# HKUST-Aerial-Robotics/ESVO

Measured on AMD Instinct MI355X. Metric: mapped events/sec (stereo TS raster + block matching + LM depth refinement + fusion), events resident in HBM before the timed region; exactly K ticks between two synchronisations, i.e. including the fill and the drain of the two-deep tick pipeline (`sustained`: the same workload over 1600 ticks), higher is better.
Workload: dtype f64

## Files before the change

esvo_amd/csrc/api_core.hip:

```cpp
#include "context.hpp"

namespace esvo_host {
thread_local std::string g_create_error;
}

namespace {

void invert3x3(const double* P, double* Kinv, double* Kinv_t) {
  const double a = P[0], b = P[1], cc = P[2], d = P[4], e = P[5], f = P[6], g = P[8], hh = P[9], i = P[10];
  const double det = a * (e * i - f * hh) - b * (d * i - f * g) + cc * (d * hh - e * g);
  const double id = 1.0 / det;
  Kinv[0] = (e * i - f * hh) * id; Kinv[1] = (cc * hh - b * i) * id; Kinv[2] = (b * f - cc * e) * id;
  Kinv[3] = (f * g - d * i) * id;  Kinv[4] = (a * i - cc * g) * id;  Kinv[5] = (cc * d - a * f) * id;
  Kinv[6] = (d * hh - e * g) * id; Kinv[7] = (b * g - a * hh) * id;  Kinv[8] = (a * e - b * d) * id;
  for (int r = 0; r < 3; ++r) Kinv_t[r] = (Kinv[r * 3 + 0] * P[3] + Kinv[r * 3 + 1] * P[7]) + Kinv[r * 3 + 2] * P[11];
}

int validate_params(const esvo_params_t* p, std::string& why) {
  if (p->ls_norm != ESVO_LSNORM_TDIST && p->ls_norm != ESVO_LSNORM_L2) { why = "LSnorm must be Tdist or l2 (DepthProblemSolver.cpp:121-131 exits on anything else)"; return ESVO_ERR_UNSUPPORTED; }
  if (p->bm_step < 1) { why = "BM_step must be >= 1"; return ESVO_ERR_INVALID_ARG; }
  if (p->patch_size_x < 1 || p->patch_size_x > 64 || p->patch_size_y < 1 || p->patch_size_y > 40) { why = "patch size must be within 1..64 x 1..40"; return ESVO_ERR_UNSUPPORTED; }
  if (p->median_blur_kernel_size < 0 || p->median_blur_kernel_size > 3) { why = "median_blur_kernel_size must be 0..3 (kernel 2k + 1)"; return ESVO_ERR_UNSUPPORTED; }
  if (p->max_event_queue_len < 0 || p->max_event_queue_len > TSQ_LMAX) { why = "max_event_queue_len must be 0 (one stamp per pixel) or 1..32"; return ESVO_ERR_UNSUPPORTED; }
  if (p->bm_max_disparity < p->bm_min_disparity || p->bm_min_disparity < 0) { why = "bad disparity range"; return ESVO_ERR_INVALID_ARG; }
// ... 26 lines not shown
  HIPCHK(hipMemsetAsync(h->d_map, 0, map_buffer_bytes(npx), st));
  HIPCHK(hipMemsetAsync(h->d_map2, 0, map_buffer_bytes(npx), st));
  HIPCHK(hipMemsetAsync(h->d_tile_count, 0, sizeof(u32) * fuse_front_tiles(h), st));
  HIPCHK(hipMemsetAsync(h->d_fuse_ctr, 0, sizeof(u32) * 2112, st));
  if (h->d_rank_kept) HIPCHK(hipMemsetAsync(h->d_rank_kept, 0, sizeof(u32) * esvo_context::SHARD_MAX_RANKS, st));
  h->d_map_cur = h->d_map;
  return ESVO_OK;
}

void read_dev_switches(esvo_context* h) {
  const char* e;
  if ((e = esvo_dev_switch("ESVO_LM_PAIR"))) h->lm_pair_forced = std::atoi(e) == 1 ? 1 : (std::atoi(e) == 0 ? 0 : -1);
  if ((e = esvo_dev_switch("ESVO_LM_QUEUES"))) h->lm_queues = std::atoi(e) == 1 ? 1 : (std::atoi(e) == 2 ? 2 : 0);
  if ((e = esvo_dev_switch("ESVO_TIMELINE"))) h->tl_on = std::atoi(e) != 0;
  if ((e = esvo_dev_switch("ESVO_LOWLAT"))) h->lat_mode = std::atoi(e) != 0;
  if ((e = esvo_dev_switch("ESVO_LOWLAT_TIMED_EVERY"))) h->lat_timed_every = std::max(1, std::atoi(e));
  if ((e = esvo_dev_switch("ESVO_REG_SPARSE"))) h->reg_sparse_forced = std::atoi(e) != 0 ? 1 : 0;
  if ((e = esvo_dev_switch("ESVO_PIPE_TIMED_EVERY"))) h->pipe_timed_every = std::max(1, std::atoi(e));
  if ((e = esvo_dev_switch("ESVO_LOWLAT_MAX_EVENTS"))) h->lat_max_events = (u32)std::strtoul(e, nullptr, 10);
  if (h->tsq_len > 0) h->tsq_tcap = (e = esvo_dev_switch("ESVO_TSQ_TILE_CAP")) ? (u32)std::max(1, std::atoi(e)) : 1024u;
  if (h->max_ev > LM_TWO_QUEUES_MAX_EVENTS && (e = esvo_dev_switch("ESVO_LM_ORDER"))) h->lm_order_on = std::atoi(e) != 0;
  if ((e = esvo_dev_switch("ESVO_BM_DEDUPE"))) h->bm_dedupe_on = std::atoi(e) != 0;
  if ((e = esvo_dev_switch("ESVO_BM_DEDUPE_MIN"))) h->bm_dedupe_min = (u32)std::max(1L, std::atol(e));
  if ((e = esvo_dev_switch("ESVO_CLK_PROBE"))) h->clk_probe = std::atoi(e) != 0;
  h->n_pose_slots = (e = esvo_dev_switch("ESVO_POSE_SLOTS0")) ? (u32)std::max(1, std::atoi(e)) : 1024u;
  if ((e = esvo_dev_switch("ESVO_FUSE_TILE_CAP"))) h->fuse_tile_cap = (u32)std::max(1L, std::atol(e));
  if ((e = esvo_dev_switch("ESVO_FUSE_PMAX"))) h->fuse_pmax_plus1 = (u32)std::max(0L, std::atol(e)) + 1u;
  if ((e = esvo_dev_switch("ESVO_FUSE_TILE_REC"))) h->fuse_tile_rec = (u32)std::max(1L, std::atol(e));
  if ((e = esvo_dev_switch("ESVO_FUSE_LDS_CAP"))) h->fuse_lds_cap = (u32)std::max(0L, std::atol(e));
}

int create_streams(esvo_context* h) {
  int prio_lo = 0, prio_hi = 0;
  CK(hipDeviceGetStreamPriorityRange(&prio_lo, &prio_hi));
  CK(hipStreamCreateWithPriority(&h->stream, hipStreamNonBlocking, prio_hi));
  CK(hipStreamCreateWithPriority(&h->stream_b, hipStreamNonBlocking, prio_hi));
  h->own_stream = true;
  CK(hipStreamCreateWithPriority(&h->stream_l, hipStreamNonBlocking, prio_lo));
  CK(hipStreamCreateWithPriority(&h->stream_l1, hipStreamNonBlocking, prio_lo));
  CK(hipStreamCreateWithFlags(&h->stream_t, hipStreamNonBlocking));
  CK(hipStreamCreateWithFlags(&h->stream_i, hipStreamNonBlocking));
  return ESVO_OK;
}

int alloc_camera(esvo_context* h, int cam, const esvo_calib_t* c) {
  const size_t npx = (size_t)h->W * h->H;
// ... 52 lines not shown
  h->d_pose_T = h->pose[0].d_T;
  return ESVO_OK;
}

int alloc_tick_scratch(esvo_context* h) {
  const size_t npx = (size_t)h->W * h->H, E = h->max_ev;
  if (h->max_ev > 4000000u) FAIL(ESVO_ERR_CAPACITY, "max_events_per_tick too large (scan limit 4M)");
  if (npx > 4000000u) FAIL(ESVO_ERR_CAPACITY, "image too large (scan limit 4M pixels)");
  CK(h->d_tick_ev.alloc(E));
  CK(h->d_match_slots.alloc(E));
  CK(h->d_match_flags.alloc(E)); CK(h->d_match_prefix.alloc(E));
  for (int k = 0; k < 2; ++k) CK(h->front[k].d_matches.alloc(E));
  if (E >= LM_SPLIT_MIN_EVENTS) {
    CK(h->d_lm_fvec0.alloc(E * 7 * 16)); CK(h->d_lm_fnorm0.alloc(E));
    CK(h->d_lm_meta.alloc(E)); CK(h->d_lm_order.alloc(E));
    CK(h->d_lm_hist.alloc(2 * 32 * 64));
    CK(hipMemset(h->d_lm_hist, 0, sizeof(u32) * 2 * 32 * 64));
  }
  if (E > LM_TWO_QUEUES_MAX_EVENTS) {
    for (int k = 0; k < 2; ++k) { CK(h->front[k].d_lm_pix_order.alloc(E)); CK(h->d_lm_sort_rows[k].alloc(E)); }
    CK(h->d_lm_sort_hist.alloc(voxel_hist_words(E)));
  }
  if (h->bm_dedupe_on && E >= h->bm_dedupe_min) CK(h->d_bm_dedupe.alloc(npx + 4 + 2 * E));
  CK(h->d_clk.alloc(2 * clk_words(h->max_ev)));
  CK(hipMemset(h->d_clk, 0, sizeof(u64) * 2 * clk_words(h->max_ev)));
  int khz = 0;
  if (hipDeviceGetAttribute(&khz, hipDeviceAttributeWallClockRate, h->device) != hipSuccess || khz <= 0) khz = 100000;
  h->stats.clk_ref_khz = (uint32_t)khz;
  for (int k = 0; k < 2; ++k) {
    CK(h->front[k].d_pt_slots.alloc(E));
    CK(h->front[k].d_pt_flags.alloc(E)); CK(h->front[k].d_pt_prefix.alloc(E));
    CK(h->front[k].d_scan_tmp_l.alloc(scan_scratch_elems(std::max(E, npx)) + 8));
  }
  CK(h->d_pts_tmp.alloc(E));
  for (int k = 0; k < 2; ++k) CK(h->front[k].d_stage.alloc(E));
  for (int k = 0; k < 2; ++k) CK(h->front[k].d_counters.alloc(CNT_ROW));
  for (int k = 0; k < 2; ++k) CK(hipMemset(h->front[k].d_counters, 0, sizeof(u32) * CNT_ROW));
  CK(h->h_counters.alloc(CNT_ROW * 2));
  std::memset(h->h_counters, 0, sizeof(u32) * CNT_ROW * 2);
  CK(h->h_pin.alloc(2 * ((size_t)h->max_poses * 17 + 16)));
  CK(h->d_scan_tmp.alloc(scan_scratch_elems(std::max(E, npx)) + 8)); CK(h->d_scan_tmp_b.alloc(scan_scratch_elems(std::max(E, npx)) + 8));
  CK(h->d_cnt_b.alloc(CNTB_ROW)); CK(hipMemset(h->d_cnt_b, 0, sizeof(u32) * CNTB_ROW));
  CK(h->h_cnt_b.alloc(CNTB_ROW * CNTB_ROWS));
  std::memset(h->h_cnt_b, 0, sizeof(u32) * CNTB_ROW * CNTB_ROWS);
  for (int k = 0; k < 2; ++k) { h->front[k].d_clk = h->d_clk + (size_t)k * clk_words(h->max_ev); h->front[k].h_counters = h->h_counters + CNT_ROW * k; h->back[k].h_cnt = h->h_cnt_b + CNTB_ROW * k; }
  CK(h->d_halo_viol.alloc(2));
// ... 367 lines not shown
```

esvo_amd/csrc/api_dev.hip:

```cpp
#include <vector>

#include "context.hpp"
#include "fdiv.hpp"

namespace {
using esvo::u32;

constexpr size_t GUARD_WORDS = 64;
constexpr size_t GUARD_BYTES = GUARD_WORDS * sizeof(u32);
constexpr u32 GUARD_PATTERN = 0xA55AC33Cu;

struct GBuf {
  uint8_t* base = nullptr;
  size_t bytes = 0;
  bool pinned = false;
  GBuf() = default;
  GBuf(const GBuf&) = delete;
  GBuf& operator=(const GBuf&) = delete;
  ~GBuf() {
    if (!base) return;
    if (pinned) hipHostFree(base);
    else hipFree(base);
  }
  hipError_t make(size_t n, const void* init, bool pin = false) {
// ... 237 lines not shown
  HIPCHK(d_r.make(img_bytes, img.data()));
  for (int k = 0; k < 2; ++k) HIPCHK(d_rows[k].make(max_matches * 8, nullptr));
  HIPCHK(d_hist.make(esvo::voxel_hist_words(max_matches) * 4, nullptr));
  HIPCHK(d_tmp.make(esvo::scan_scratch_elems(esvo::voxel_hist_words(max_matches)) * 4, nullptr));
  HIPCHK(d_order.make(max_matches * 4, order));
  esvo::DevParams dp;
  std::memset(&dp, 0, sizeof(dp));
  dp.W = width; dp.H = height; dp.num_threads = num_threads; dp.updown = updown;
  esvo::u64* const rows[2] = {d_rows[0].ptr<esvo::u64>(), d_rows[1].ptr<esvo::u64>()};
  esvo::launch_lm_pixel_order(d_m.ptr<esvo_match_t>(), d_n.ptr<u32>(), cap, 0, d_l.ptr<uint8_t>(), d_r.ptr<uint8_t>(), dp, rows,
                              d_hist.ptr<u32>(), d_tmp.ptr<u32>(), d_order.ptr<u32>(), st.s);
  DEV_RUN_DONE();
  HIPCHK(d_m.finish(nullptr, &bad));
  HIPCHK(d_n.finish(nullptr, &bad));
  HIPCHK(d_l.finish(nullptr, &bad));
  HIPCHK(d_r.finish(nullptr, &bad));
  for (int k = 0; k < 2; ++k) HIPCHK(d_rows[k].finish(nullptr, &bad));
  HIPCHK(d_hist.finish(nullptr, &bad));
  HIPCHK(d_tmp.finish(nullptr, &bad));
  HIPCHK(d_order.finish(order, &bad));
  DEV_RETURN();
}

int esvo_debug_upload_words(const void* src, size_t bytes, void* dst, uint32_t* zero, uint32_t zero_words, uint32_t n_zero) {
  if (bytes % 4 || (bytes && (!src || !dst)) || n_zero > 256u || (zero ? n_zero > zero_words : n_zero != 0)) return ESVO_ERR_INVALID_ARG;
  DEV_BEGIN();
  GBuf h_src, d_dst, d_zero;
  HIPCHK(h_src.make(bytes, src, true));
  HIPCHK(d_dst.make(bytes, dst));
  if (zero) HIPCHK(d_zero.make((size_t)zero_words * 4, zero));
  esvo::launch_upload_words(h_src.ptr<void>(), d_dst.ptr<void>(), bytes, st.s, zero ? d_zero.ptr<u32>() : nullptr, n_zero);
  DEV_RUN_DONE();
  HIPCHK(h_src.finish(nullptr, &bad));
  HIPCHK(d_dst.finish(dst, &bad));
  if (zero) HIPCHK(d_zero.finish(zero, &bad));
  DEV_RETURN();
}

int esvo_debug_back_prologue(const void* src, size_t bytes, void* dst, const void* a_src, size_t a_bytes, void* a_dst, size_t a_dst_bytes,
                             const void* b_src, size_t b_bytes, void* b_dst, const uint32_t* a_flags, const uint32_t* a_prefix,
                             uint32_t a_slots) {
  if (bytes % 4 || a_bytes % 8 || b_bytes % 8 || a_dst_bytes % 8) return ESVO_ERR_INVALID_ARG;
  if ((bytes && (!src || !dst)) || (a_bytes && !a_src) || (a_dst_bytes && !a_dst) || (b_bytes && (!b_src || !b_dst))) return ESVO_ERR_INVALID_ARG;
  if (a_flags ? (!a_prefix || a_bytes != (size_t)a_slots * sizeof(esvo_depth_point_t)) : (a_dst_bytes != a_bytes)) return ESVO_ERR_INVALID_ARG;
  if (a_flags) {
    for (u32 i = 0; i < a_slots; ++i)
// ... 105 lines not shown
  HIPCHK(hipSetDevice(h->device));
  int rc = flush_pending_tick(h);
  if (rc) return rc;
  rc = drain_lm_and_back(h);
  if (rc) return rc;
  HIPCHK(hipMemcpy(out, h->d_cell_count, sizeof(u32) * n, hipMemcpyDeviceToHost));
  return ESVO_OK;
}

int esvo_debug_bm_owner_count(esvo_handle h, uint32_t* n_owners, int* shared) {
  if (!h || !n_owners || !shared) return ESVO_ERR_INVALID_ARG;
  API_LOCK(h);
  HIPCHK(hipSetDevice(h->device));
  int rc = flush_pending_tick(h);
  if (rc) return rc;
  *n_owners = 0;
  *shared = h->d_bm_dedupe ? 1 : 0;
  if (!h->d_bm_dedupe) return ESVO_OK;
  HIPCHK(hipStreamSynchronize(h->stream));
  HIPCHK(hipMemcpy(n_owners, h->d_bm_dedupe + (size_t)h->W * h->H, sizeof(u32), hipMemcpyDeviceToHost));
  return ESVO_OK;
}

void esvo_debug_live_allocations(size_t out[2]) {
  out[0] = esvo::g_live_allocs.load();
  out[1] = esvo::g_live_bytes.load();
}

int esvo_debug_devmem_selftest(int pinned) { return pinned ? devmem_selftest<true>() : devmem_selftest<false>(); }

}
```

esvo_amd/csrc/api_map.hip:

```cpp
#include "context.hpp"

namespace esvo_host {

u64 lower_bound_sec(const esvo_context* h, int cam, double t) {
  const auto& v = h->ts_host[cam];
  size_t lo = 0, hi = v.size();
  while (lo < hi) {
    size_t mid = (lo + hi) / 2;
    if (ns_to_sec(v[mid]) < t) lo = mid + 1; else hi = mid;
  }
  return h->ring_base[cam] + lo;
}
u64 ros_time_from_sec(double t) {
  long long sec64 = (long long)std::floor(t);
  u32 sec = (u32)sec64;
  u32 nsec = (u32)std::round((t - sec) * 1e9);
  sec += (nsec / 1000000000ul);
  nsec %= 1000000000ul;
  return (u64)sec * 1000000000ull + nsec;
}

int upload_poses(esvo_context* h, const uint64_t* pose_t_ns, const double* pose_T, size_t m, u32* d_zero_row) {
  if (m > h->max_poses) FAIL(ESVO_ERR_CAPACITY, "pose table larger than max_poses_per_tick");
  h->pin_slot ^= 1;
// ... 2 lines not shown
  double* sec = pin + 16 * m;
  for (size_t i = 0; i < m; ++i) sec[i] = ns_to_sec(pose_t_ns[i]);
  std::memcpy(T, pose_T, sizeof(double) * 16 * m);
  h->h_pose_T.assign(pose_T, pose_T + 16 * m);
  h->n_pose = (u32)m;
  h->pose_buf ^= 1;
  h->d_pose_T = h->pose[h->pose_buf].d_T;
  HIPCHK(hipStreamWaitEvent(h->stream, h->pose[h->pose_buf].released, 0));
  h->d_pose_sec = h->d_pose_T + 16 * m;
  launch_upload_words(T, h->d_pose_T, sizeof(double) * 17 * m, h->stream, d_zero_row, CNT_ROW);
  return ESVO_OK;
}

int run_bm(esvo_context* h, const esvo_event_t* d_ev, u64 first, u64 cap, int reverse, u32 n, const u32* sel) {
  FrontSlot& F = h->front_cur();
  BmArgs a;
  a.ev = d_ev; a.n = n; a.ev_first = first; a.ev_cap = cap; a.ev_reverse = reverse; a.sel = sel;
  a.tsL = h->d_obs[0]; a.tsR = h->d_obs[1];
  a.lut = h->d_lut; a.mask = h->d_mask;
  a.pose_sec = h->d_pose_sec; a.n_pose = h->n_pose;
  a.out_slots = h->d_match_slots; a.out_flags = h->d_match_flags;
  a.fail_counters = F.d_counters;
  if (h->stage_events_on) hipEventRecord(F.ev->e[FE_BM0], h->stream);
  if (h->d_bm_dedupe && n >= h->bm_dedupe_min && n <= h->max_ev && !h->sharded && bm_dedupe_applies(a, h->dp)) {
    u32* owner = h->d_bm_dedupe;
    u32* n_uniq = owner + (size_t)h->W * h->H;
    u32* uniq_w = n_uniq + 4;
    launch_bm_match_dedupe(a, h->dp, owner, uniq_w, n_uniq, uniq_w + h->max_ev, h->stream);
  } else {
    launch_bm_match(a, h->dp, h->stream);
  }
  if (h->stage_events_on) hipEventRecord(F.ev->e[FE_BM1], h->stream);
  HIPCHK(hipGetLastError());
  return ESVO_OK;
}
int run_order_matches(esvo_context* h, u32 n, bool local, bool by_index) {
  FrontSlot& F = h->front_cur();
  if (scan_compact_is_small(n)) {
    by_index = by_index && !local;
    launch_scan_compact_matches_small(h->d_match_flags, h->d_match_prefix, F.d_counters + (local ? CNT_OWN_MATCHES : CNT_MATCHES), n, h->d_match_slots,
                                      by_index ? nullptr : F.d_matches, (local || by_index) ? h->d_own_w : nullptr, h->stream);
  } else {
    launch_exclusive_scan_u32(h->d_match_flags, h->d_match_prefix, F.d_counters + (local ? CNT_OWN_MATCHES : CNT_MATCHES), h->d_scan_tmp, n, h->stream);
    launch_compact_matches(h->d_match_slots, h->d_match_flags, h->d_match_prefix, n, F.d_matches, local ? h->d_own_w : nullptr,
                           h->stream);
  }
  if (h->stage_events_on) hipEventRecord(F.ev->e[FE_S1], h->stream);
// ... 594 lines not shown
```

esvo_amd/csrc/common.hpp:

```cpp
#pragma once

#include <hip/hip_runtime.h>
#include <stdint.h>

#include "../../include/esvo_hip.h"

#define ESVO_WAVE 64

#include <cstdlib>
#include <cstring>
inline const char* esvo_dev_switch(const char* name) {
  const char* on = std::getenv("ESVO_DEV_SWITCHES");
  return (on && std::strcmp(on, "1") == 0) ? std::getenv(name) : nullptr;
}

namespace esvo {

typedef unsigned long long u64;
typedef unsigned int u32;

struct CamConst {
  double P[12];
  double Kinv[9];
  double Kinv_t[3];
// ... 154 lines not shown
  u64* q;
  int L;
  u32* tcount; uint4* tlist; u32 tcap;
  uint4* over; u32* over_count; u32 over_cap;
};
void launch_tsq_insert(const TsQueueArgs& a, int W, int H, hipStream_t s);
void launch_tsq_view(const u64* q, int L, int W, int H, u64 t_ns, u64* sae, hipStream_t s);
struct TsPair { const u64* sae[2]; uint8_t* raw[2]; const int2* fixmap[2]; uint8_t* out[2]; uint8_t* out2[2]; };
void launch_ts_scatter_segs(const TsScatterSegs& g, int n_seg, int W, int H, hipStream_t s);
void launch_ts_render_pair(const TsPair& c, int W, int H, u64 t_ns, double decay_sec, int ignore_polarity, int median_k,
                           hipStream_t s, int row0 = 0, int row1 = -1);
void launch_ts_render_forward(const u64* d_sae, const u32* d_off, const u32* d_src, const float2* d_lut, double* d_val,
                              uint8_t* d_raw, uint8_t* d_out, int W, int H, u64 t_ns, double decay_sec, int ignore_polarity,
                              int median_k, hipStream_t s);
void launch_gaussian5_pair(const uint8_t* in0, const uint8_t* in1, uint8_t* out0, uint8_t* out1, int W, int H, hipStream_t s,
                           int row0 = 0, int row1 = -1);
void launch_denoise_flags(const esvo_event_t* ring, u64 first, u64 cap, u32 n, uint8_t* evmap, u32* flags, int W, int H,
                          hipStream_t s);
void launch_denoise_select(const u32* flags, const u32* prefix, u32 n, u32* sel, hipStream_t s);
void launch_denoise_bits_routed(const esvo_event_t* ring, u64 first, u64 cap, u32 n_loc, const u32* gidx, u32 g_first, u32 n, uint8_t* evmap,
                                int W, int H, int band_y0, int band_y1, u32* bits, hipStream_t s);
void launch_denoise_bits_unpack(const u32* blocks, u32 block_words, u32 N, u32 n, u32* flags, hipStream_t s);

struct BmArgs {
  const esvo_event_t* ev;
  u32 n;
  u64 ev_first;
  u64 ev_cap;
  int ev_reverse;
  const u32* sel;
  const uint8_t* tsL;
  const uint8_t* tsR;
  const float2* lut;
  const uint8_t* mask;
  const double* pose_sec;
  u32 n_pose;
  esvo_match_t* out_slots;
  u32* out_flags;
  u32* fail_counters;
  const u32* gidx = nullptr;
  u32 g_first = 0;
  u32 n_loc = 0;
  const u32* keep_flags = nullptr;
  const u32* keep_prefix = nullptr;
  u32 n_raw = 0;
  const u32* uniq_w = nullptr;
  const u32* n_uniq = nullptr;
  u32* search_rec = nullptr;
};
void launch_bm_match(const BmArgs& a, const DevParams& p, hipStream_t s);
constexpr unsigned long long BM_LDS_MAX_BYTES = 160ull * 1024ull;
unsigned long long bm_match_lds_bytes(int wx, int wy, int dmin, int dmax, int step, int updown);
constexpr u32 BM_DEDUPE_MIN_EVENTS = 40001u;
bool bm_dedupe_applies(const BmArgs& a, const DevParams& p);
void launch_bm_match_dedupe(BmArgs a, const DevParams& p, u32* owner, u32* uniq_w, u32* n_uniq, u32* search_rec, hipStream_t s);
void launch_compact_matches(const esvo_match_t* slots, const u32* flags, const u32* prefix, u32 n,
                            esvo_match_t* out, u32* slot_of, hipStream_t s);
void launch_matches_to_points(const esvo_match_t* m, const u32* n_ptr, u32 max_n, esvo_depth_point_t* out, const DevParams& p,
                              hipStream_t s);

struct TrackRef { double T[16]; };
struct TrackPose { double T[16]; double Jc[6]; };
#define TRK_NE_MAX_POSES 4
struct TrackPoseSet { TrackPose p[TRK_NE_MAX_POSES]; };
struct TrackArgs {
  const double* pts;
  const uint8_t* neg;
  const int16_t* du;
  const int16_t* dv;
  const uint8_t* mask;
  double P[12];
  int W, H;
};
void launch_track_images(const uint8_t* blurred, uint8_t* neg, int16_t* du, int16_t* dv, int W, int H, hipStream_t s);
void launch_track_reference(const float* xyz, u32 n, const TrackRef& r, double* pts, hipStream_t s);
void launch_track_reference_gather(const float* cloud_xyz, const u32* order, u32 n, const TrackRef& r, double* pts, hipStream_t s);
void launch_track_residuals(const TrackArgs& a, const TrackPose& pose, u32 offset, u32 count, int huber, double thr, double* fvec,
                            hipStream_t s);
// ... 162 lines not shown
```

esvo_amd/csrc/context.hpp:

```cpp
#pragma once
#include <algorithm>
#include <array>
#include <atomic>
#include <chrono>
#include <cmath>
#include <cstdio>
#include <cstdlib>
#include <cstring>
#include <deque>
#include <mutex>
#include <string>
#include <vector>

#include "common.hpp"
#include "devmem.hpp"

using namespace esvo;

struct FrameRec {
  u32 off;
  u32 count;
  u32 slot;
  u32 run;
};
// ... 165 lines not shown
  DevBuf<uint8_t> d_wire[2];
  u64 ring_cap = 0;
  DevEvent evt_ingest[2];

  DevBuf<uint8_t> d_obs_tmp;

  PoseBuf pose[2];
  int pose_buf = 0;
  std::vector<double> h_pose_T;
  PinBuf<double> h_pin;

  u32 max_ev = 0;
  DevBuf<esvo_event_t> d_tick_ev;
  DevBuf<esvo_match_t> d_match_slots;
  DevBuf<u32> d_match_flags, d_match_prefix;
  DevBuf<double> d_lm_fvec0, d_lm_fnorm0;
  DevBuf<u32> d_lm_meta, d_lm_order, d_lm_hist;
  DevBuf<u64> d_lm_sort_rows[2];
  DevBuf<u32> d_lm_sort_hist;
  bool lm_order_on = true;
  DevBuf<u32> d_bm_dedupe;
  bool bm_dedupe_on = true;
  u32 bm_dedupe_min = esvo::BM_DEDUPE_MIN_EVENTS;
  DevBuf<u64> d_clk;
  bool clk_probe = true;
  DevBuf<DevPoint> d_pts_tmp;
  PinBuf<u32> h_counters;
  DevBuf<u32> d_scan_tmp;
  DevBuf<u32> d_cnt_b;
  PinBuf<u32> h_cnt_b;
  DevBuf<u32> d_scan_tmp_b;

  DevBuf<DevPoint> d_win;
  u32 win_cap = 0;
  u32 n_pose_slots = 0;
  std::vector<char> slot_used;
  DevBuf<double> d_frame_pose_T;
  u32 max_poses = 0;
  DevBuf<u32> d_fr_table;
  PinBuf<u32> h_fr_table;
  u32 max_frames = 0;

  DevBuf<DevPoint> d_prop;
  DevBuf<u32> d_tile_count;
  DevBuf<uint2> d_tile_pts, d_over_pts;
  DevBuf<u32> d_cell_count, d_cell_offset, d_cell_list;
// ... 229 lines not shown
```

esvo_amd/csrc/kernels_bm.hip:

```cpp
#include "common.hpp"
#include "fdiv.hpp"

namespace esvo {

__device__ inline int wave_sum_i32(int v) {
#pragma unroll
  for (int d = 32; d >= 1; d >>= 1) v += __shfl_xor(v, d, ESVO_WAVE);
  return v;
}
__device__ inline long long wave_sum_i64(long long v) {
#pragma unroll
  for (int d = 32; d >= 1; d >>= 1) v += __shfl_xor(v, d, ESVO_WAVE);
  return v;
}

typedef u32 u32x4_a4 __attribute__((ext_vector_type(4), aligned(4)));

struct ZnccLeft {
  double sigl;
  int Sl;
};
__device__ inline double sqrt_var(double v) { return v > 0 ? sqrt_moderate(v) : 0.0; }
__device__ inline ZnccLeft zncc_left(int Sl, int Sll, int N, const Recip& rn2) {
  ZnccLeft z;
  z.Sl = Sl;
  z.sigl = sqrt_var(div_fast((double)(N * Sll - Sl * Sl), rn2)) + 1e-6;
  return z;
}
__device__ inline double zncc_from_moments(const ZnccLeft& zl, int Sr, int Srr, int Slr, int N, const Recip& rn,
                                           const Recip& rn2) {
  const double varr = div_fast((double)(N * Srr - Sr * Sr), rn2);
  const double sigr = sqrt_var(varr) + 1e-6;
  const double cov = div_fast((double)(N * Slr - zl.Sl * Sr), rn);
  Recip rs;
  rs.b = zl.sigl * sigr;
  rs.y = recip_refined(rs.b);
  return 0.5 * (1 - div_fast(div_fast(cov, rs), rn));
}

extern __shared__ __attribute__((aligned(16))) unsigned char bm_smem[];

template <int G>
__device__ inline int grp_sum_i32(int v) {
#pragma unroll
  for (int d = G / 2; d >= 1; d >>= 1) v += __shfl_xor(v, d, G);
  return v;
}

#ifndef BM_BLOCK
#define BM_BLOCK 64
#endif

__device__ inline uint4 load_row15(const u32* ts32, int n_dw, int A) {
  const int a0 = A >> 2;
  const u32 sh = (u32)(A & 3);
  u32 d[5];
#pragma unroll
  for (int j = 0; j < 5; ++j) {
    int idx = a0 + j;
    idx = idx < 0 ? 0 : (idx >= n_dw ? n_dw - 1 : idx);
    d[j] = ts32[idx];
// ... 25 lines not shown
  e = reinterpret_cast<const uint4*>(a.ev)[ei];
}

template <int G>
__device__ inline void grp_argmin(double& best, int& bestd) {
#pragma unroll
  for (int s = G / 2; s >= 1; s >>= 1) {
    const double oc = __shfl_xor(best, s, G);
    const int od = __shfl_xor(bestd, s, G);
    if (od >= 0 && (bestd < 0 || oc < best || (oc == best && od > bestd))) { best = oc; bestd = od; }
  }
}

__device__ inline u32 pose_lower_bound(const BmArgs& a, const uint4& e) {
  const double te = time_to_sec(e.y, e.z);
  u32 lo = 0, hi = a.n_pose;
  while (lo < hi) {
    const u32 mid = (lo + hi) >> 1;
    if (a.pose_sec[mid] < te) lo = mid + 1; else hi = mid;
  }
  return lo;
}

template <int G, bool COARSE, bool UPDOWN>
__global__ void __launch_bounds__(BM_BLOCK) bm_match_kernel(BmArgs a, DevParams p, int RD, int lds_per_event) {
  constexpr int EPB = BM_BLOCK / G;
  const int grp = threadIdx.x / G, l = threadIdx.x % G;
  const u32 pos = blockIdx.x * EPB + grp;
  const u32 n_out = a.gidx ? a.n_loc : a.n;
  u32 w = a.gidx ? pos : pos * (u32)p.ev_nshards + (u32)p.ev_shard;
  if (a.uniq_w) {
    const u32 nu = *a.n_uniq;
    if (blockIdx.x * EPB >= nu) return;
    w = pos < nu ? a.uniq_w[pos] : n_out;
  }
  u32* ldsL = reinterpret_cast<u32*>(bm_smem + grp * lds_per_event);
  u32* ldsR = ldsL + 28;
  const int nd = p.dmax - p.dmin + 1;
  double* cost_row = reinterpret_cast<double*>(ldsR + (UPDOWN ? (nd + 6) * 4 : 7 * RD));

  const int W = p.W, H = p.H;
  constexpr int wx = 15, wy = 7, N = wx * wy, hx = 7, hy = 3;

  bool ok = w < n_out;
  u32 k = 0;
  uint4 e = make_uint4(0, 0, 0, 0);
  if (ok) bm_item(a, p, w, k, e, ok);
  const int ex = e.x & 0xffffu, ey = e.x >> 16;
  double xr = 0, yr = 0;
  int x1 = 0, y1 = 0;
  if (ok) ok = ex < W && ey < H;
  if (ok) {
    const float2 q = a.lut[ey * W + ex];
    xr = (double)q.x;
    yr = (double)q.y;
    ok = !(xr < 0 || xr > (double)(W - 1) || yr < 0 || yr > (double)(H - 1));
    if (a.gidx && ok) { const int yb = (int)floor(yr); ok = yb >= p.band_y0 && yb < p.band_y1; }
  }
  if (ok && a.mask) ok = a.mask[(int)yr * W + (int)xr] > 125;
  if (ok) {
    x1 = (int)floor(xr);
    y1 = (int)floor(yr);
  }
  if (ok) ok = !(x1 - hx < 1 || y1 - hy < 1 || x1 + hx >= W - 1 || y1 + hy >= H - 1);
  int reason = 0;

  int Sl = 0, Sll = 0;
  if (ok) {
    int cnt = 0, sl = 0, sll = 0;
    if (l < wy) {
      const u32* ts32 = reinterpret_cast<const u32*>(a.tsL);
      const int n_dw = (W * H + 3) >> 2;
      const uint4 wv = load_row15(ts32, n_dw, (y1 - hy + l) * W + (x1 - hx));
      *reinterpret_cast<uint4*>(ldsL + l * 4) = wv;
      u32 usl = 0, usll = 0;
      usl = __builtin_amdgcn_udot4(wv.x, 0x01010101u, usl, false);
      usl = __builtin_amdgcn_udot4(wv.y, 0x01010101u, usl, false);
      usl = __builtin_amdgcn_udot4(wv.z, 0x01010101u, usl, false);
      usl = __builtin_amdgcn_udot4(wv.w, 0x01010101u, usl, false);
      usll = __builtin_amdgcn_udot4(wv.x, wv.x, usll, false);
      usll = __builtin_amdgcn_udot4(wv.y, wv.y, usll, false);
      usll = __builtin_amdgcn_udot4(wv.z, wv.z, usll, false);
      usll = __builtin_amdgcn_udot4(wv.w, wv.w, usll, false);
      auto zero_bytes = [](u32 x) {
        return __popc(~(((x & 0x7f7f7f7fu) + 0x7f7f7f7fu) | x | 0x7f7f7f7fu));
      };
      cnt = zero_bytes(wv.x) + zero_bytes(wv.y) + zero_bytes(wv.z) + zero_bytes(wv.w | 0xff000000u);
      sl = (int)usl;
// ... 37 lines not shown
          *reinterpret_cast<uint4*>(ldsR + py * RD + 4 * j4) = v;
        }
      }
    }
  }
  __syncthreads();

  auto cand_valid = [&](int d) {
    if constexpr (UPDOWN) { const int y2 = y1 - d; return !(y2 - hy < 1 || y2 + hy >= H - 1); }
    else { const int x2 = x1 - d; return !(x2 - hx < 1 || x2 + hx >= W - 1); }
  };
  double best = 1.0;
  int bestd = -1;
  if (ok) {
    const Recip rn = make_recip((double)N), rn2 = make_recip((double)N * (double)N);
    const ZnccLeft zl = zncc_left(Sl, Sll, N, rn2);
    u32 L[wy][4];
#pragma unroll
    for (int py = 0; py < wy; ++py) {
      const uint4 v = *reinterpret_cast<const uint4*>(ldsL + py * 4);
      L[py][0] = v.x; L[py][1] = v.y; L[py][2] = v.z; L[py][3] = v.w;
    }
    for (int d = p.dmin + l; d <= p.dmax; d += G) {
      if (!cand_valid(d)) {
        if constexpr (COARSE) cost_row[d - p.dmin] = 1.0;
        continue;
      }
      const int col0 = p.dmax - d;
      u32 sr = 0, srr = 0, slr = 0;
#pragma unroll
      for (int py = 0; py < wy; ++py) {
        u32 w0, w1, w2, w3;
        if constexpr (UPDOWN) {
          const uint4 v = *reinterpret_cast<const uint4*>(ldsR + (col0 + py) * 4);
          w0 = v.x; w1 = v.y; w2 = v.z; w3 = v.w;
        } else {
          const int b = o_row[py] + col0;
          const u32* row = ldsR + py * RD + (b >> 2);
          const u32 sh = (u32)(b & 3);
          const u32 d0 = row[0], d1 = row[1], d2 = row[2], d3 = row[3], d4 = row[4];
          w0 = __builtin_amdgcn_alignbyte(d1, d0, sh);
          w1 = __builtin_amdgcn_alignbyte(d2, d1, sh);
          w2 = __builtin_amdgcn_alignbyte(d3, d2, sh);
          w3 = __builtin_amdgcn_alignbyte(d4, d3, sh) & 0x00ffffffu;
        }
        slr = __builtin_amdgcn_udot4(L[py][0], w0, slr, false);
        slr = __builtin_amdgcn_udot4(L[py][1], w1, slr, false);
        slr = __builtin_amdgcn_udot4(L[py][2], w2, slr, false);
        slr = __builtin_amdgcn_udot4(L[py][3], w3, slr, false);
        sr = __builtin_amdgcn_udot4(w0, 0x01010101u, sr, false);
        sr = __builtin_amdgcn_udot4(w1, 0x01010101u, sr, false);
        sr = __builtin_amdgcn_udot4(w2, 0x01010101u, sr, false);
        sr = __builtin_amdgcn_udot4(w3, 0x01010101u, sr, false);
        srr = __builtin_amdgcn_udot4(w0, w0, srr, false);
        srr = __builtin_amdgcn_udot4(w1, w1, srr, false);
        srr = __builtin_amdgcn_udot4(w2, w2, srr, false);
        srr = __builtin_amdgcn_udot4(w3, w3, srr, false);
      }
      const double cost = zncc_from_moments(zl, (int)sr, (int)srr, (int)slr, N, rn, rn2);
      if constexpr (COARSE) cost_row[d - p.dmin] = cost;
      else if (cost <= best) { best = cost; bestd = d; }
    }
  }
  if constexpr (COARSE) {
    __syncthreads();
    if (ok) {
      const int step = p.step;
      const int nc = (p.dmax - p.dmin) / step + 1;
      for (int j = l; j < nc; j += G) {
        const int d = p.dmin + j * step;
        if (!cand_valid(d)) continue;
        const double c = cost_row[d - p.dmin];
        if (c <= best) { best = c; bestd = d; }
      }
      grp_argmin<G>(best, bestd);
      bool found = bestd >= 0 && bestd - step >= p.dmin && bestd + step <= p.dmin + (nc - 1) * step;
      if (found) found = cost_row[bestd - step - p.dmin] < 1.0 && cost_row[bestd + step - p.dmin] < 1.0 && best < p.zncc_thr;
      if (!found) { ok = false; reason = 2; }
      else {
        const int cd = bestd;
        double fb = 2.0;
        int fd = -1;
// ... 243 lines not shown
    return (unsigned long long)(((N + 7) & ~7LL) + bm_any_strip_bytes(wx, wy, nd, updown != 0) + (coarse ? nd * 8 : 0));
  }
  return (unsigned long long)(bm_15x7_event_bytes(nd, coarse, updown != 0) * (BM_BLOCK / bm_group_width(nd)));
}

template <bool COARSE, bool UPDOWN>
static void launch_bm_any(const BmArgs& a, const DevParams& p, hipStream_t s) {
  const int nd = p.dmax - p.dmin + 1;
  const int strip = (int)bm_any_strip_bytes(p.wx, p.wy, nd, UPDOWN);
  const size_t lds = (size_t)bm_match_lds_bytes(p.wx, p.wy, p.dmin, p.dmax, COARSE ? 2 : 1, UPDOWN);
  const u32 own = a.gidx ? a.n_loc : ((a.n > (u32)p.ev_shard) ? (a.n - (u32)p.ev_shard + (u32)p.ev_nshards - 1) / (u32)p.ev_nshards : 0);
  if (own == 0) return;
  hipLaunchKernelGGL((bm_match_any_kernel<COARSE, UPDOWN>), dim3(own), dim3(64), lds, s, a, p, strip);
}

template <int G, bool COARSE, bool UPDOWN>
static void launch_bm_g(const BmArgs& a, const DevParams& p, int RD, hipStream_t s) {
  const int nd = p.dmax - p.dmin + 1;
  const int per_event = (int)bm_15x7_event_bytes(nd, COARSE, UPDOWN);
  const int epb = BM_BLOCK / G;
  const u32 own = a.gidx ? a.n_loc : ((a.n > (u32)p.ev_shard) ? (a.n - (u32)p.ev_shard + (u32)p.ev_nshards - 1) / (u32)p.ev_nshards : 0);
  if (own == 0) return;
  const u32 blocks = (own + epb - 1) / epb;
  hipLaunchKernelGGL((bm_match_kernel<G, COARSE, UPDOWN>), dim3(blocks), dim3(BM_BLOCK), (size_t)per_event * epb, s, a, p, RD, per_event);
}
template <bool COARSE, bool UPDOWN>
static void launch_bm_mode(int G, const BmArgs& a, const DevParams& p, int RD, hipStream_t s) {
  switch (G) {
    case 64: launch_bm_g<64, COARSE, UPDOWN>(a, p, RD, s); break;
    case 32: launch_bm_g<32, COARSE, UPDOWN>(a, p, RD, s); break;
    case 16: launch_bm_g<16, COARSE, UPDOWN>(a, p, RD, s); break;
    default: launch_bm_g<8, COARSE, UPDOWN>(a, p, RD, s); break;
  }
}

void launch_bm_match(const BmArgs& a, const DevParams& p, hipStream_t s) {
  if (a.n == 0) return;
  const int nd = p.dmax - p.dmin + 1;
  const int RD = (int)bm_strip_dwords(nd);
  const int bestG = bm_group_width(nd);
  const bool coarse = p.step > 1;
  if (p.wx != 15 || p.wy != 7) {
    if (p.updown) { if (coarse) launch_bm_any<true, true>(a, p, s); else launch_bm_any<false, true>(a, p, s); }
    else { if (coarse) launch_bm_any<true, false>(a, p, s); else launch_bm_any<false, false>(a, p, s); }
    return;
  }
  if (p.updown) {
    if (coarse) launch_bm_mode<true, true>(bestG, a, p, RD, s);
    else launch_bm_mode<false, true>(bestG, a, p, RD, s);
  } else {
    if (coarse) launch_bm_mode<true, false>(bestG, a, p, RD, s);
    else launch_bm_mode<false, false>(bestG, a, p, RD, s);
  }
}

__global__ void __launch_bounds__(256) bm_claim_kernel(BmArgs a, DevParams p, u32* __restrict__ owner, u32* __restrict__ n_uniq) {
  const u32 w = blockIdx.x * blockDim.x + threadIdx.x;
  if (w == 0) *n_uniq = 0u;
  if (w >= a.n) return;
  u32 k = 0;
  uint4 e;
  bool ok = true;
  bm_item(a, p, w, k, e, ok);
  const int ex = e.x & 0xffffu, ey = e.x >> 16;
  if (ex < p.W && ey < p.H) atomicMin(owner + ey * p.W + ex, w);
}
__global__ void __launch_bounds__(256) bm_owner_list_kernel(BmArgs a, DevParams p, const u32* __restrict__ owner, u32* __restrict__ uniq_w,
                                                            u32* __restrict__ n_uniq) {
  __shared__ u32 wave_cnt[4];
  __shared__ u32 base;
  const u32 w = blockIdx.x * blockDim.x + threadIdx.x;
  bool own = false;
  if (w < a.n) {
    u32 k = 0;
    uint4 e;
    bool ok = true;
// ... 113 lines not shown
```

esvo_amd/lib.py:

```python
import ctypes as C
import os
import subprocess

import numpy as np

from .abi import (DEPTH_POINT_DTYPE, EM_POSE_FN, ERR_CAPACITY, ERR_INVALID_ARG, ERR_STATE, EVENT_DTYPE, MATCH_DTYPE, CalibStruct, EmSelectionStruct,
                  EmStatsStruct, GpcParamsStruct, GpcStatsStruct, ParamsStruct, SgmStatsStruct, StatsStruct, TRACK_ITER_DTYPE, TRACK_SOLVE_MAX_ITERATIONS,
                  TrackSolveInfoStruct, TrackSolveParamsStruct)

_CSRC = os.path.join(os.path.dirname(os.path.abspath(__file__)), "csrc")
_LIB_PATH = os.environ.get("ESVO_HIP_LIB") or os.path.join(_CSRC, "libesvo_hip.so")
_SOURCES = ["api_core.hip", "api_ts.hip", "api_map.hip", "api_window.hip", "api_modes.hip", "api_shard.hip", "api_out.hip", "api_comm.hip", "api_bag.hip", "api_track.hip", "scan.hip", "kernels_ts.hip", "kernels_bm.hip", "kernels_lm.hip", "kernels_lm_any.hip", "kernels_fuse.hip", "kernels_shard.hip", "kernels_track.hip", "kernels_track_viz.hip", "kernels_viz.hip", "kernels_sgm.hip", "api_em.hip", "kernels_em.hip", "kernels_cloud.hip", "api_dev.hip", "api_gpc.hip", "kernels_voxel.hip", "api_history.hip"]
HIPCC_FLAGS = ["--offload-arch=gfx950", "-O3", "-std=c++17", "-ffp-contract=off", "-fPIC", "-shared",
               "-Wno-unused-value", "-Wno-unused-result", "-ldl"]

SYMBOLS = [
    "esvo_default_params", "esvo_create", "esvo_destroy", "esvo_reset", "esvo_set_params", "esvo_last_error",
    "esvo_set_stream", "esvo_synchronize", "esvo_ts_push_events", "esvo_ts_push_events_async", "esvo_ts_push_wait", "esvo_host_alloc", "esvo_host_free", "esvo_ts_push_event_array", "esvo_ts_render", "esvo_ts_render_forward", "esvo_map_set_observation",
    "esvo_map_match", "esvo_map_set_poses", "esvo_map_refine", "esvo_map_push_frame", "esvo_map_fuse",
    "esvo_map_tick", "esvo_map_tick_bm_only", "esvo_map_fuse_matches_naive", "esvo_map_tick_resident", "esvo_map_get_depth_points", "esvo_map_get_committed", "esvo_map_get_pointcloud_xyz", "esvo_map_get_last_frame",
    "esvo_get_stats", "esvo_shard_set_band", "esvo_shard_set_routing", "esvo_shard_get_rows", "esvo_shard_exchange", "esvo_shard_tick_phase", "esvo_abi_sizes",
    "esvo_map_front", "esvo_map_front_frame", "esvo_map_push_frame_device", "esvo_map_fuse_async",
    "esvo_track_set_current", "esvo_track_get_images", "esvo_track_set_reference", "esvo_track_residuals", "esvo_track_jacobian",
    "esvo_track_normal_equations", "esvo_track_normal_equations_batch", "esvo_track_register", "esvo_track_solve", "esvo_track_sizes",
# ... 370 lines not shown
    n = len(flags)
    prefix, total = _prefilled(n, np.uint32), _prefilled(1, np.uint32)
    out = _prefilled(n, MATCH_DTYPE) if want_out else None
    slot_of = _prefilled(n, np.uint32) if want_slot_of else None
    fn = _dbg_fn("esvo_debug_compact_matches", [C.c_void_p, C.c_size_t] + [C.c_void_p] * 5)
    g = _dbg_rc(fn(flags.ctypes.data, n, slots.ctypes.data, prefix.ctypes.data, total.ctypes.data, _p(out), _p(slot_of)),
                "esvo_debug_compact_matches")
    return dict(prefix=prefix, total=int(total[0]), out=out, slot_of=slot_of, guards=g)


def debug_lm_order(matches, max_matches, width, height, left, right, num_threads=1, updown=False):
    matches = _dbg_array(matches, MATCH_DTYPE, "matches")
    left = _dbg_array(np.asarray(left).reshape(-1), np.uint8, "left", width * height)
    right = _dbg_array(np.asarray(right).reshape(-1), np.uint8, "right", width * height)
    order = _prefilled(max_matches, np.uint32)
    variant = C.c_int(-1)
    fn = _dbg_fn("esvo_debug_lm_order", [C.c_void_p, C.c_size_t, C.c_size_t, C.c_int, C.c_int, C.c_int, C.c_int, C.c_void_p, C.c_void_p,
                                         C.c_void_p, C.c_void_p])
    g = _dbg_rc(fn(matches.ctypes.data if len(matches) else None, len(matches), int(max_matches), int(width), int(height), int(num_threads),
                   1 if updown else 0, left.ctypes.data, right.ctypes.data, order.ctypes.data, C.addressof(variant)), "esvo_debug_lm_order")
    return dict(order=order, variant=int(variant.value), guards=g)


def debug_compact_points(flags, slots, want_out=True, row=None, total_index=0, pinned_row=False):
    flags, slots = _check_compact_args(flags, slots, DEPTH_POINT_DTYPE)
    n = len(flags)
    if row is None and pinned_row:
        raise ValueError("pinned_row needs the device row it mirrors")
    if row is not None:
        row = _dbg_array(row, np.uint32, "row").copy()
        if not 0 <= total_index < len(row) <= 1024:
            raise ValueError("total_index must lie inside the row (at most 1024 words)")
    prefix, total = _prefilled(n, np.uint32), _prefilled(1, np.uint32)
    out = _prefilled(n, DEPTH_POINT_DTYPE) if want_out else None
    row_host = _prefilled(len(row), np.uint32) if pinned_row else None
    fn = _dbg_fn("esvo_debug_compact_points", [C.c_void_p, C.c_size_t] + [C.c_void_p] * 5 + [C.c_uint32, C.c_uint32, C.c_void_p])
    g = _dbg_rc(fn(flags.ctypes.data, n, slots.ctypes.data, prefix.ctypes.data, None if row is not None else total.ctypes.data, _p(out),
                   _p(row), 0 if row is None else len(row), int(total_index), _p(row_host)), "esvo_debug_compact_points")
    return dict(prefix=prefix, total=int(total[0]) if row is None else int(row[total_index]), out=out, row=row, row_host=row_host,
                guards=g)


def debug_upload_words(src, zero_words=None, n_zero=0):
    src = _dbg_array(src, np.uint32, "src")
    if not 0 <= n_zero <= 256 or n_zero > (zero_words or 0):
        raise ValueError("n_zero: at most 256 words, inside the zero buffer")
# ... 441 lines not shown
        st = np.ascontiguousarray(stamps, np.uint64)
        T = np.ascontiguousarray(poses, np.float64).reshape(-1, 16)
        Tw = np.ascontiguousarray(T_world_cam, np.float64).reshape(16)
        self._ck(self.lib.esvo_map_tick_resident(self.h, int(t_ns), Tw.ctypes.data, st.ctypes.data, T.ctypes.data, st.shape[0]))

    def get_map(self):
        n = C.c_size_t(0)
        out = np.zeros(self.W * self.H, DEPTH_POINT_DTYPE)
        self._ck(self.lib.esvo_map_get_depth_points(self.h, out.ctypes.data, out.shape[0], C.byref(n)))
        return out[: n.value].copy()

    def debug_fuse_cell_counts(self):
        out = np.zeros((self.H, self.W), np.uint32)
        fn = _dbg_fn("esvo_debug_fuse_cell_counts", [C.c_void_p, C.c_void_p, C.c_size_t])
        self._ck(fn(self.h, out.ctypes.data, out.size))
        return out

    def debug_bm_owner_count(self):
        n, shared = C.c_uint32(0), C.c_int(0)
        fn = _dbg_fn("esvo_debug_bm_owner_count", [C.c_void_p, C.c_void_p, C.c_void_p])
        self._ck(fn(self.h, C.byref(n), C.byref(shared)))
        return int(n.value) if shared.value else None

    def get_committed_map(self):
        out = np.zeros(self.W * self.H, DEPTH_POINT_DTYPE)
        n, t = C.c_size_t(), C.c_uint64()
        self._ck(self.lib.esvo_map_get_committed(self.h, out.ctypes.data, out.shape[0], C.byref(n), C.byref(t)))
        return out[:n.value].copy(), int(t.value)

    def get_pointcloud(self):
        n = C.c_size_t(0)
        out = np.zeros((self.W * self.H, 3), np.float32)
        self._ck(self.lib.esvo_map_get_pointcloud_xyz(self.h, out.ctypes.data, out.shape[0], C.byref(n)))
        return out[: n.value].copy()

    def map_cloud_build(self):
        n = C.c_size_t(0)
        self._ck(self.lib.esvo_map_cloud_build(self.h, C.byref(n)))
        return int(n.value)

    def map_cloud(self):
        n = C.c_size_t(0)
        self._ck(self.lib.esvo_map_cloud_get(self.h, None, 0, C.byref(n)))
        out = np.zeros((int(n.value), 3), np.float32)
        if n.value:
            self._ck(self.lib.esvo_map_cloud_get(self.h, out.ctypes.data, out.shape[0], C.byref(n)))
# ... 287 lines not shown
```

Baseline: 188.1 million.

## Precompute right-image patch moments per pixel for block matching

Adds a per-pixel kernel that computes each right-image patch's sum and standard deviation once per tick using sliding row sums, and stores them in a 16-byte table. The block-matching kernel then reads one record per candidate disparity, prefetching the next one, instead of recomputing the right-patch sum and sum of squares with udot4 for every event and candidate. This removes redundant per-candidate arithmetic, including a sqrt, at the cost of an extra full-image pass and a 16-byte gather per candidate. It is enabled by default above a minimum event count. The moments kernel hardcodes a 15x7 patch.

```diff
diff --git a/esvo_amd/csrc/api_core.hip b/esvo_amd/csrc/api_core.hip
--- a/esvo_amd/csrc/api_core.hip
+++ b/esvo_amd/csrc/api_core.hip
@@ -72,6 +72,8 @@
   if (h->max_ev > LM_TWO_QUEUES_MAX_EVENTS && (e = esvo_dev_switch("ESVO_LM_ORDER"))) h->lm_order_on = std::atoi(e) != 0;
   if ((e = esvo_dev_switch("ESVO_BM_DEDUPE"))) h->bm_dedupe_on = std::atoi(e) != 0;
   if ((e = esvo_dev_switch("ESVO_BM_DEDUPE_MIN"))) h->bm_dedupe_min = (u32)std::max(1L, std::atol(e));
+  if ((e = esvo_dev_switch("ESVO_BM_MOMENTS"))) h->bm_moments_on = std::atoi(e) != 0;
+  if ((e = esvo_dev_switch("ESVO_BM_MOMENTS_MIN"))) h->bm_moments_min = (u32)std::max(1L, std::atol(e));
   if ((e = esvo_dev_switch("ESVO_CLK_PROBE"))) h->clk_probe = std::atoi(e) != 0;
   h->n_pose_slots = (e = esvo_dev_switch("ESVO_POSE_SLOTS0")) ? (u32)std::max(1, std::atoi(e)) : 1024u;
   if ((e = esvo_dev_switch("ESVO_FUSE_TILE_CAP"))) h->fuse_tile_cap = (u32)std::max(1L, std::atol(e));
@@ -170,6 +172,7 @@
     CK(h->d_lm_sort_hist.alloc(voxel_hist_words(E)));
   }
   if (h->bm_dedupe_on && E >= h->bm_dedupe_min) CK(h->d_bm_dedupe.alloc(npx + 4 + 2 * E));
+  if (h->bm_moments_on && E >= h->bm_moments_min) CK(h->d_bm_rmom.alloc(npx));
   CK(h->d_clk.alloc(2 * clk_words(h->max_ev)));
   CK(hipMemset(h->d_clk, 0, sizeof(u64) * 2 * clk_words(h->max_ev)));
   int khz = 0;
diff --git a/esvo_amd/csrc/api_dev.hip b/esvo_amd/csrc/api_dev.hip
--- a/esvo_amd/csrc/api_dev.hip
+++ b/esvo_amd/csrc/api_dev.hip
@@ -283,6 +283,25 @@
   DEV_RETURN();
 }
 
+int esvo_debug_bm_right_moments(const uint8_t* right, int width, int height, double* sig_r, int32_t* Sr) {
+  if (!right || !sig_r || !Sr || width < 1 || height < 1 || (size_t)width * height > 4000000u) return ESVO_ERR_INVALID_ARG;
+  DEV_BEGIN();
+  GBuf d_r, d_out;
+  const size_t npx = (size_t)width * height, img_bytes = (npx + 3) / 4 * 4;
+  std::vector<uint8_t> img(img_bytes, 0);
+  std::memcpy(img.data(), right, npx);
+  HIPCHK(d_r.make(img_bytes, img.data()));
+  std::vector<esvo::BmRight> rec(npx);
+  for (size_t i = 0; i < npx; ++i) { rec[i].sig_r = sig_r[i]; rec[i].Sr = Sr[i]; rec[i].pad = (int)GUARD_PATTERN; }
+  HIPCHK(d_out.make(npx * sizeof(esvo::BmRight), rec.data()));
+  esvo::launch_bm_right_moments(d_r.ptr<uint8_t>(), width, height, d_out.ptr<esvo::BmRight>(), st.s);
+  DEV_RUN_DONE();
+  HIPCHK(d_r.finish(nullptr, &bad));
+  HIPCHK(d_out.finish(rec.data(), &bad));
+  for (size_t i = 0; i < npx; ++i) { sig_r[i] = rec[i].sig_r; Sr[i] = rec[i].Sr; bad += (rec[i].pad != 0); }
+  DEV_RETURN();
+}
+
 int esvo_debug_upload_words(const void* src, size_t bytes, void* dst, uint32_t* zero, uint32_t zero_words, uint32_t n_zero) {
   if (bytes % 4 || (bytes && (!src || !dst)) || n_zero > 256u || (zero ? n_zero > zero_words : n_zero != 0)) return ESVO_ERR_INVALID_ARG;
   DEV_BEGIN();
@@ -434,6 +453,13 @@
   return ESVO_OK;
 }
 
+int esvo_debug_bm_moments_used(esvo_handle h, int* used) {
+  if (!h || !used) return ESVO_ERR_INVALID_ARG;
+  API_LOCK(h);
+  *used = h->bm_moments_used ? 1 : 0;
+  return ESVO_OK;
+}
+
 void esvo_debug_live_allocations(size_t out[2]) {
   out[0] = esvo::g_live_allocs.load();
   out[1] = esvo::g_live_bytes.load();
diff --git a/esvo_amd/csrc/api_map.hip b/esvo_amd/csrc/api_map.hip
--- a/esvo_amd/csrc/api_map.hip
+++ b/esvo_amd/csrc/api_map.hip
@@ -48,7 +48,13 @@
   a.out_slots = h->d_match_slots; a.out_flags = h->d_match_flags;
   a.fail_counters = F.d_counters;
   if (h->stage_events_on) hipEventRecord(F.ev->e[FE_BM0], h->stream);
-  if (h->d_bm_dedupe && n >= h->bm_dedupe_min && n <= h->max_ev && !h->sharded && bm_dedupe_applies(a, h->dp)) {
+  const bool slice = n <= h->max_ev && !h->sharded && bm_dedupe_applies(a, h->dp);
+  h->bm_moments_used = h->d_bm_rmom && n >= h->bm_moments_min && slice;
+  if (h->bm_moments_used) {
+    launch_bm_right_moments(a.tsR, h->dp.W, h->dp.H, h->d_bm_rmom, h->stream);
+    a.rmom = h->d_bm_rmom;
+  }
+  if (h->d_bm_dedupe && n >= h->bm_dedupe_min && slice) {
     u32* owner = h->d_bm_dedupe;
     u32* n_uniq = owner + (size_t)h->W * h->H;
     u32* uniq_w = n_uniq + 4;
diff --git a/esvo_amd/csrc/common.hpp b/esvo_amd/csrc/common.hpp
--- a/esvo_amd/csrc/common.hpp
+++ b/esvo_amd/csrc/common.hpp
@@ -200,6 +200,12 @@
                                 int W, int H, int band_y0, int band_y1, u32* bits, hipStream_t s);
 void launch_denoise_bits_unpack(const u32* blocks, u32 block_words, u32 N, u32 n, u32* flags, hipStream_t s);
 
+struct alignas(16) BmRight {
+  double sig_r;
+  int Sr;
+  int pad;
+};
+static_assert(sizeof(BmRight) == 16, "one 16-byte load per candidate");
 struct BmArgs {
   const esvo_event_t* ev;
   u32 n;
@@ -225,6 +231,7 @@
   const u32* uniq_w = nullptr;
   const u32* n_uniq = nullptr;
   u32* search_rec = nullptr;
+  const BmRight* rmom = nullptr;
 };
 void launch_bm_match(const BmArgs& a, const DevParams& p, hipStream_t s);
 constexpr unsigned long long BM_LDS_MAX_BYTES = 160ull * 1024ull;
@@ -232,6 +239,8 @@
 constexpr u32 BM_DEDUPE_MIN_EVENTS = 40001u;
 bool bm_dedupe_applies(const BmArgs& a, const DevParams& p);
 void launch_bm_match_dedupe(BmArgs a, const DevParams& p, u32* owner, u32* uniq_w, u32* n_uniq, u32* search_rec, hipStream_t s);
+constexpr u32 BM_MOMENTS_MIN_EVENTS = 40001u;
+void launch_bm_right_moments(const uint8_t* tsR, int W, int H, BmRight* out, hipStream_t s);
 void launch_compact_matches(const esvo_match_t* slots, const u32* flags, const u32* prefix, u32 n,
                             esvo_match_t* out, u32* slot_of, hipStream_t s);
 void launch_matches_to_points(const esvo_match_t* m, const u32* n_ptr, u32 max_n, esvo_depth_point_t* out, const DevParams& p,
diff --git a/esvo_amd/csrc/context.hpp b/esvo_amd/csrc/context.hpp
--- a/esvo_amd/csrc/context.hpp
+++ b/esvo_amd/csrc/context.hpp
@@ -211,6 +211,10 @@
   DevBuf<u32> d_bm_dedupe;
   bool bm_dedupe_on = true;
   u32 bm_dedupe_min = esvo::BM_DEDUPE_MIN_EVENTS;
+  DevBuf<esvo::BmRight> d_bm_rmom;
+  bool bm_moments_on = true;
+  u32 bm_moments_min = esvo::BM_MOMENTS_MIN_EVENTS;
+  bool bm_moments_used = false;
   DevBuf<u64> d_clk;
   bool clk_probe = true;
   DevBuf<DevPoint> d_pts_tmp;
diff --git a/esvo_amd/csrc/kernels_bm.hip b/esvo_amd/csrc/kernels_bm.hip
--- a/esvo_amd/csrc/kernels_bm.hip
+++ b/esvo_amd/csrc/kernels_bm.hip
@@ -37,6 +37,13 @@
   rs.y = recip_refined(rs.b);
   return 0.5 * (1 - div_fast(div_fast(cov, rs), rn));
 }
+__device__ inline double zncc_from_table(const ZnccLeft& zl, int Sr, double sigr, int Slr, int N, const Recip& rn) {
+  const double cov = div_fast((double)(N * Slr - zl.Sl * Sr), rn);
+  Recip rs;
+  rs.b = zl.sigl * sigr;
+  rs.y = recip_refined(rs.b);
+  return 0.5 * (1 - div_fast(div_fast(cov, rs), rn));
+}
 
 extern __shared__ __attribute__((aligned(16))) unsigned char bm_smem[];
 
@@ -108,7 +115,7 @@
   return lo;
 }
 
-template <int G, bool COARSE, bool UPDOWN>
+template <int G, bool COARSE, bool UPDOWN, bool RMOM = false>
 __global__ void __launch_bounds__(BM_BLOCK) bm_match_kernel(BmArgs a, DevParams p, int RD, int lds_per_event) {
   constexpr int EPB = BM_BLOCK / G;
   const int grp = threadIdx.x / G, l = threadIdx.x % G;
@@ -150,6 +157,14 @@
   }
   if (ok) ok = !(x1 - hx < 1 || y1 - hy < 1 || x1 + hx >= W - 1 || y1 + hy >= H - 1);
   int reason = 0;
+  auto rm_index = [&](int d) {
+    const int i = UPDOWN ? (y1 - d) * p.W + x1 : y1 * p.W + (x1 - d);
+    return min(max(i, 0), p.W * p.H - 1);
+  };
+  BmRight rm_next;
+  if constexpr (RMOM) {
+    if (ok) rm_next = a.rmom[rm_index(p.dmin + l)];
+  }
 
   int Sl = 0, Sll = 0;
   if (ok) {
@@ -233,6 +248,11 @@
       L[py][0] = v.x; L[py][1] = v.y; L[py][2] = v.z; L[py][3] = v.w;
     }
     for (int d = p.dmin + l; d <= p.dmax; d += G) {
+      BmRight rm;
+      if constexpr (RMOM) {
+        rm = rm_next;
+        rm_next = a.rmom[rm_index(d + G)];
+      }
       if (!cand_valid(d)) {
         if constexpr (COARSE) cost_row[d - p.dmin] = 1.0;
         continue;
@@ -259,16 +279,20 @@
         slr = __builtin_amdgcn_udot4(L[py][1], w1, slr, false);
         slr = __builtin_amdgcn_udot4(L[py][2], w2, slr, false);
         slr = __builtin_amdgcn_udot4(L[py][3], w3, slr, false);
-        sr = __builtin_amdgcn_udot4(w0, 0x01010101u, sr, false);
-        sr = __builtin_amdgcn_udot4(w1, 0x01010101u, sr, false);
-        sr = __builtin_amdgcn_udot4(w2, 0x01010101u, sr, false);
-        sr = __builtin_amdgcn_udot4(w3, 0x01010101u, sr, false);
-        srr = __builtin_amdgcn_udot4(w0, w0, srr, false);
-        srr = __builtin_amdgcn_udot4(w1, w1, srr, false);
-        srr = __builtin_amdgcn_udot4(w2, w2, srr, false);
-        srr = __builtin_amdgcn_udot4(w3, w3, srr, false);
-      }
-      const double cost = zncc_from_moments(zl, (int)sr, (int)srr, (int)slr, N, rn, rn2);
+        if constexpr (!RMOM) {
+          sr = __builtin_amdgcn_udot4(w0, 0x01010101u, sr, false);
+          sr = __builtin_amdgcn_udot4(w1, 0x01010101u, sr, false);
+          sr = __builtin_amdgcn_udot4(w2, 0x01010101u, sr, false);
+          sr = __builtin_amdgcn_udot4(w3, 0x01010101u, sr, false);
+          srr = __builtin_amdgcn_udot4(w0, w0, srr, false);
+          srr = __builtin_amdgcn_udot4(w1, w1, srr, false);
+          srr = __builtin_amdgcn_udot4(w2, w2, srr, false);
+          srr = __builtin_amdgcn_udot4(w3, w3, srr, false);
+        }
+      }
+      double cost;
+      if constexpr (RMOM) cost = zncc_from_table(zl, rm.Sr, rm.sig_r, (int)slr, N, rn);
+      else cost = zncc_from_moments(zl, (int)sr, (int)srr, (int)slr, N, rn, rn2);
       if constexpr (COARSE) cost_row[d - p.dmin] = cost;
       else if (cost <= best) { best = cost; bestd = d; }
     }
@@ -558,7 +582,10 @@
   const u32 own = a.gidx ? a.n_loc : ((a.n > (u32)p.ev_shard) ? (a.n - (u32)p.ev_shard + (u32)p.ev_nshards - 1) / (u32)p.ev_nshards : 0);
   if (own == 0) return;
   const u32 blocks = (own + epb - 1) / epb;
-  hipLaunchKernelGGL((bm_match_kernel<G, COARSE, UPDOWN>), dim3(blocks), dim3(BM_BLOCK), (size_t)per_event * epb, s, a, p, RD, per_event);
+  if (a.rmom)
+    hipLaunchKernelGGL((bm_match_kernel<G, COARSE, UPDOWN, true>), dim3(blocks), dim3(BM_BLOCK), (size_t)per_event * epb, s, a, p, RD, per_event);
+  else
+    hipLaunchKernelGGL((bm_match_kernel<G, COARSE, UPDOWN>), dim3(blocks), dim3(BM_BLOCK), (size_t)per_event * epb, s, a, p, RD, per_event);
 }
 template <bool COARSE, bool UPDOWN>
 static void launch_bm_mode(int G, const BmArgs& a, const DevParams& p, int RD, hipStream_t s) {
@@ -588,6 +615,52 @@
     if (coarse) launch_bm_mode<true, false>(bestG, a, p, RD, s);
     else launch_bm_mode<false, false>(bestG, a, p, RD, s);
   }
+}
+
+constexpr int BM_RM_ROWS = 8;
+__global__ void __launch_bounds__(64) bm_right_moments_kernel(const uint8_t* __restrict__ tsR, int W, int H, BmRight* __restrict__ out) {
+  constexpr int N = 15 * 7, hx = 7, hy = 3, K = BM_RM_ROWS;
+  const int x = blockIdx.x * 64 + threadIdx.x, y0 = blockIdx.y * K;
+  if (x >= W) return;
+  const u32* ts32 = reinterpret_cast<const u32*>(tsR);
+  const int n_dw = (W * H + 3) >> 2;
+  int hs[K + 6], hq[K + 6];
+#pragma unroll
+  for (int r = 0; r < K + 6; ++r) {
+    const uint4 wv = load_row15(ts32, n_dw, (y0 - hy + r) * W + (x - hx));
+    u32 s = 0, q = 0;
+    s = __builtin_amdgcn_udot4(wv.x, 0x01010101u, s, false);
+    s = __builtin_amdgcn_udot4(wv.y, 0x01010101u, s, false);
+    s = __builtin_amdgcn_udot4(wv.z, 0x01010101u, s, false);
+    s = __builtin_amdgcn_udot4(wv.w, 0x01010101u, s, false);
+    q = __builtin_amdgcn_udot4(wv.x, wv.x, q, false);
+    q = __builtin_amdgcn_udot4(wv.y, wv.y, q, false);
+    q = __builtin_amdgcn_udot4(wv.z, wv.z, q, false);
+    q = __builtin_amdgcn_udot4(wv.w, wv.w, q, false);
+    hs[r] = (int)s;
+    hq[r] = (int)q;
+  }
+  const Recip rn2 = make_recip((double)N * (double)N);
+  const bool x_ok = !(x - hx < 1 || x + hx >= W - 1);
+#pragma unroll
+  for (int i = 0; i < K; ++i) {
+    const int y = y0 + i;
+    if (y >= H) break;
+    int Sr = 0, Srr = 0;
+#pragma unroll
+    for (int k = 0; k < 7; ++k) { Sr += hs[i + k]; Srr += hq[i + k]; }
+    const double sig = sqrt_var(div_fast((double)(N * Srr - Sr * Sr), rn2)) + 1e-6;
+    const bool valid = x_ok && !(y - hy < 1 || y + hy >= H - 1);
+    BmRight r;
+    r.sig_r = valid ? sig : 0.0;
+    r.Sr = valid ? Sr : 0;
+    r.pad = 0;
+    out[(size_t)y * W + x] = r;
+  }
+}
+void launch_bm_right_moments(const uint8_t* tsR, int W, int H, BmRight* out, hipStream_t s) {
+  if (W < 1 || H < 1) return;
+  hipLaunchKernelGGL(bm_right_moments_kernel, dim3((W + 63) / 64, (H + BM_RM_ROWS - 1) / BM_RM_ROWS), dim3(64), 0, s, tsR, W, H, out);
 }
 
 __global__ void __launch_bounds__(256) bm_claim_kernel(BmArgs a, DevParams p, u32* __restrict__ owner, u32* __restrict__ n_uniq) {
diff --git a/esvo_amd/lib.py b/esvo_amd/lib.py
--- a/esvo_amd/lib.py
+++ b/esvo_amd/lib.py
@@ -416,6 +416,18 @@
     return dict(order=order, variant=int(variant.value), guards=g)
 
 
+def debug_bm_right_moments(right):
+    right = np.asarray(right)
+    if right.dtype != np.uint8 or right.ndim != 2:
+        raise ValueError(f"right: an (H, W) uint8 image is expected, not {right.dtype} with {right.ndim} axes")
+    right = np.ascontiguousarray(right)
+    H, W = right.shape
+    sig, sr = _prefilled(H * W, np.float64), _prefilled(H * W, np.int32)
+    fn = _dbg_fn("esvo_debug_bm_right_moments", [C.c_void_p, C.c_int, C.c_int, C.c_void_p, C.c_void_p])
+    g = _dbg_rc(fn(right.ctypes.data, W, H, sig.ctypes.data, sr.ctypes.data), "esvo_debug_bm_right_moments")
+    return sig.reshape(H, W), sr.reshape(H, W), g
+
+
 def debug_compact_points(flags, slots, want_out=True, row=None, total_index=0, pinned_row=False):
     flags, slots = _check_compact_args(flags, slots, DEPTH_POINT_DTYPE)
     n = len(flags)
@@ -903,6 +915,12 @@
         self._ck(fn(self.h, C.byref(n), C.byref(shared)))
         return int(n.value) if shared.value else None
 
+    def debug_bm_moments_used(self):
+        used = C.c_int(0)
+        fn = _dbg_fn("esvo_debug_bm_moments_used", [C.c_void_p, C.c_void_p])
+        self._ck(fn(self.h, C.byref(used)))
+        return bool(used.value)
+
     def get_committed_map(self):
         out = np.zeros(self.W * self.H, DEPTH_POINT_DTYPE)
         n, t = C.c_size_t(), C.c_uint64()
```

Result: slower. 185.5 million (-1.4%).
